# Prasaya/brax

Measured on AMD Instinct MI355X. Metric: env-steps/sec (Ant, 4096 envs/GPU), higher is better.
Workload: dtype f32

## Files before the change

brax_amd/csrc/bx_mix.h:

```cpp
#pragma once
#include <hip/hip_runtime.h>
#include <stdint.h>

namespace bx {

__host__ __device__ __forceinline__ uint64_t mix64(uint64_t seed, uint64_t i) {
  uint64_t z = seed * 0x9E3779B97F4A7C15ull + i + 0x632BE59BD9B4E019ull;
  z = (z ^ (z >> 30)) * 0xBF58476D1CE4E5B9ull;
  z = (z ^ (z >> 27)) * 0x94D049BB133111EBull;
  return z ^ (z >> 31);
}

}
```

brax_amd/csrc/pbd_kernels.hip:

```cpp
#pragma once
#include <hip/hip_runtime.h>
#include <stdint.h>
#include <stdlib.h>
#include <string.h>

#include <type_traits>

#include "bx_mix.h"
#include "pbd_features.h"
#include "pbd_launch.h"
#include "pbd_layout.h"
#include "pbd_math.h"
#include "pbd_stamps.h"

namespace bx {

struct Cst {
  const uint32_t* __restrict__ w;
  __device__ __forceinline__ int i(int off) const { return (int)w[off]; }
  __device__ __forceinline__ float f(int off) const { return __uint_as_float(w[off]); }
  __device__ __forceinline__ v3 f3(int off) const { return mk(f(off), f(off + 1), f(off + 2)); }
};

struct BodyC {
// ... 3399 lines not shown
      for (; i < e && (c.i(H.o_cl + i) >> 24) == g; i++) {
        const float* s = E.cslot + (c.i(H.o_cl + i) & 0xFFFFFF) * SLOT_STRIDE;
        gv = gv + ld3(s);
        ga = ga + ld3(s + 3);
        cnt += s[7];
      }
      float d = 1e-8f + cnt;
      dv = dv + gv / d;
      da = da + ga / d;
    }
    float* acc = E.acc + b * ACC_STRIDE;
    st3(acc + ACC_ICV, dv);
    st3(acc + ACC_ICA, da);
  }
  esync<L>();
}


template <int L>
__device__ void joint_angles(const Cst& c, const BlobHdr& H, const Env& E, int lane,
                             const JointC* hj = nullptr) {
  for (int j = lane; j < H.J; j += L) {
    JointC Jc = hj ? *hj : load_joint(c, H, j);
    QP p = ldqp(E.qp + Jc.bp * QP_STRIDE), q = ldqp(E.qp + Jc.bc * QP_STRIDE);
    v3 axes[3];
    float ang[3];
    axis_angle<F_ALL>(Jc, p, q, axes, ang);
    v3 dv = p.ang - q.ang;
#pragma unroll
    for (int l = 0; l < 3; l++) {
      if (l < Jc.n_angles) {
        E.ang[Jc.angle_off + l] = ang[l];
        E.ang[H.D + Jc.angle_off + l] = dot(dv, axes[l]);
      }
    }
  }
}

__device__ __forceinline__ float clip1(float x) { return clampn(x, -1.f, 1.f); }

__device__ __forceinline__ float euler_z(const float* q) {
  return atan2f(-2.f * q[1] * q[2] + 2.f * q[0] * q[3],
                q[1] * q[1] + q[0] * q[0] - q[3] * q[3] - q[2] * q[2]);
}

__device__ __forceinline__ float euler_y(const float* q) {
  return asinf(clampn(2.f * q[1] * q[3] + 2.f * q[0] * q[2], -1.f, 1.f));
}

__device__ void humanoid_com(const Cst& c, const BlobHdr& H, const float* qp, v3& com, float& msum,
                             bool n16 = false, const float* lmass = nullptr) {
  v3 acc = mk(0.f, 0.f, 0.f);
  float m = 0.f;
  if (n16) {
#pragma unroll
    for (int b = 0; b < 16; b++) {
      const bool in = b < H.N - 1;
      const int bb = in ? b : 0;
      const float w = in ? (lmass ? lmass[bb] : c.f(H.o_body + bb * BODY_STRIDE + BODY_MASS)) : 0.f;
      acc = acc + w * ld3(qp + bb * QP_STRIDE);
      m += w;
    }
    com = acc / m;
    msum = m;
    return;
  }
  for (int b = 0; b < H.N - 1; b++) {
    float mb = c.f(H.o_body + b * BODY_STRIDE + BODY_MASS);
    acc = acc + mb * ld3(qp + b * QP_STRIDE);
    m += mb;
  }
  com = acc / m;
  msum = m;
}

template <int EK>
__device__ __forceinline__ constexpr bool ek_has(int k) {
  return EK == EK_ANY || (EK == EK_ANT && k == BX_ENV_ANT) ||
         (EK == EK_HUM && (k == BX_ENV_HUMANOID || k == BX_ENV_HUMANOID_STANDUP)) ||
         (EK == EK_CHEETAH && k == BX_ENV_HALFCHEETAH) || (EK == EK_PUSHER && k == BX_ENV_PUSHER);
}
#define KIND_IS(k) (ek_has<EK>(k) && kind == (k))

__device__ __forceinline__ float uniform_at(uint64_t seed, uint64_t i, float lo, float hi) {
  const uint64_t z = mix64(seed, i);
  float u = (float)(z >> 40) * (1.0f / 16777216.0f);
  return lo + (hi - lo) * u;
}

__device__ __forceinline__ void arm_tip(const Env& E, const float* coef, v3& tp, v3& tv) {
  const float* a = E.qp + (int)coef[1] * QP_STRIDE;
  v3 off = rotate(mk(.11f, 0.f, 0.f), q4{a[3], a[4], a[5], a[6]});
  tp = ld3(a) + off;
  tv = ld3(a + 7) + cross(ld3(a + 10), off);
}

template <int EK>
__device__ float obs_elem(const Cst& c, const BlobHdr& H, const Env& E, int kind, int flags, int i,
                          const float* act, int aw, bool valid, const float* coef) {
  const int N = H.N, D = H.D;
  const float* q0 = E.qp;
  const bool loco2d = KIND_IS(BX_ENV_HOPPER) || KIND_IS(BX_ENV_WALKER2D);
  if (flags & BX_OBS_XY) {
    if (KIND_IS(BX_ENV_HALFCHEETAH) || loco2d) {
      if (i == 0) return q0[0];
      i -= 1;
    } else {
      if (i < 2) return q0[i];
      i -= 2;
    }
  }
  if (KIND_IS(BX_ENV_ANT)) {
    if (i == 0) return q0[2];
    i -= 1;
    if (i < 4) return q0[3 + i];
    i -= 4;
    if (i < D) return E.ang[i];
    i -= D;
    if (i < 3) return q0[7 + i];
    i -= 3;
    if (i < 3) return q0[10 + i];
    i -= 3;
    if (i < D) return E.ang[D + i];
    i -= D;
    if (i < 3 * N) return clip1(E.acc[(i / 3) * ACC_STRIDE + ACC_ICV + i % 3]);
    i -= 3 * N;
    return clip1(E.acc[(i / 3) * ACC_STRIDE + ACC_ICA + i % 3]);
  }
  if (loco2d) {
    if (i == 0) return q0[2];
    if (i == 1) return euler_y(q0 + 3);
    i -= 2;
    if (i < D) return E.ang[i];
    i -= D;
    if (i == 0) return q0[7];
    if (i == 1) return q0[9];
    if (i == 2) return q0[11];
    i -= 3;
    return E.ang[D + i];
  }
  if (KIND_IS(BX_ENV_INVERTED_PENDULUM)) {
    if (i == 0) return q0[0];
    i -= 1;
    if (i < D) return E.ang[i];
    i -= D;
    if (i == 0) return q0[7];
    return E.ang[D + i - 1];
  }
  if (KIND_IS(BX_ENV_INVERTED_DOUBLE_PENDULUM)) {
    if (i == 0) return q0[0];
    i -= 1;
    if (i < D) return sinf(E.ang[i]);
    i -= D;
    if (i < D) return cosf(E.ang[i]);
    i -= D;
    if (i == 0) return q0[7];
    return E.ang[D + i - 1];
  }
  if (KIND_IS(BX_ENV_ACROBOT)) return E.ang[i];
  if (KIND_IS(BX_ENV_REACHER) || KIND_IS(BX_ENV_REACHERANGLE)) {
    if (i < D) return cosf(E.ang[i]);
    i -= D;
    if (i < D) return sinf(E.ang[i]);
    i -= D;
    const float* tq = E.qp + (int)coef[0] * QP_STRIDE;
    if (i < 2) return tq[i];
    i -= 2;
    v3 tp, tv;
    arm_tip(E, coef, tp, tv);
    if (i < 2) return i == 0 ? tv.x : tv.y;
// ... 201 lines not shown
          o[k] = clip1(a[ACC_ICV + k]);
          o[3 * N + k] = clip1(a[ACC_ICA + k]);
        }
      }
    return;
  }
  if constexpr (EK == EK_HUM && L <= 64) {
    const int N = H.N, D = H.D, M = N - 1;
    const int x = (flags & BX_OBS_XY) ? 2 : 0;
    const float* q0 = E.qp;
    for (int l = lane; l < x + 11; l += L) {
      const int k = l - x;
      float v = l < x ? q0[l] : (k < 5 ? q0[2 + k] : q0[7 + (k - 5)]);
      obs_out[k < 5 ? l : x + 5 + D + (k - 5)] = v;
    }
    for (int j = lane; j < D; j += L) {
      obs_out[x + 5 + j] = E.ang[j];
      obs_out[x + 11 + D + j] = E.ang[D + j];
    }
    const int base = x + 11 + 2 * D;
    const v3 com = ld3(E.red + 32);
    const float msum = E.red[35];
    BX_OST(2);
    for (int b = lane; b < M; b += L) {
      const int ob = H.o_body + b * BODY_STRIDE;
      const float mb = hbody ? hbody->mass : c.f(ob + BODY_MASS);
      const float Ia[3] = {hbody ? hbody->I.x : c.f(ob + BODY_I),
                           hbody ? hbody->I.y : c.f(ob + BODY_I + 1),
                           hbody ? hbody->I.z : c.f(ob + BODY_I + 2)};
      const v3 d = ld3(E.qp + b * QP_STRIDE) - com;
      const v3 vb = ld3(E.qp + b * QP_STRIDE + 7);
      const float nn = norm(d);
      const float dd[3] = {d.x, d.y, d.z};
      float* o = obs_out + base + 9 * b;
#pragma unroll
      for (int r = 0; r < 3; r++)
#pragma unroll
        for (int cc = 0; cc < 3; cc++) {
          float v = mb * (float)(r == cc) * (nn * nn);
          v += (r == cc ? Ia[r] : 0.f) - dd[r] * dd[cc];
          o[3 * r + cc] = v;
        }
      float* ov = obs_out + base + 9 * M + 3 * b;
      ov[0] = mb * vb.x / msum;
      ov[1] = mb * vb.y / msum;
      ov[2] = mb * vb.z / msum;
      const v3 cr = cross(d, vb);
      const float den = 1e-7f + nn * nn;
      float* oa = obs_out + base + 12 * M + 3 * b;
      oa[0] = cr.x / den;
      oa[1] = cr.y / den;
      oa[2] = cr.z / den;
    }
    BX_OST(3);
    const bool ha = lane < H.K;
    ActC A{};
    int dof = 0;
    if (ha && hact && hj) {
      A = *hact;
      dof = hj->dof;
    } else if (ha) {
      A = load_act(c, H, lane);
      dof = c.i(H.o_joint + A.joint * JOINT_STRIDE + J_DOF);
    }
    int off = dof;
    constexpr int W = L < 64 ? L : 64;
#pragma unroll
    for (int sh = 1; sh < W; sh <<= 1) {
      int t = __shfl_up(off, sh, W);
      if ((lane % W) >= sh) off += t;
    }
    off -= dof;
    float* oq = obs_out + base + 15 * M + off;
#pragma unroll
    for (int i = 0; i < 3; i++)
      if (i < dof) oq[i] = (act ? E.arow[take_idx(A.idx[i], aw)] : 0.f) * A.strength;
    BX_OST(4);
    return;
  }
  for (int i = lane; i < obs_size; i += L)
    obs_out[i] = obs_elem<EK>(c, H, E, kind, flags, i, act, aw, act != nullptr, coef);
}




#if defined(BX_WAVES1)
#define BX_STEP_ATTR __attribute__((amdgpu_waves_per_eu(1, 1)))
#else
#define BX_STEP_ATTR
#endif

template <int MODE>
__device__ __forceinline__ float* stage_constants(const uint32_t* blob, const BlobHdr& H,
                                                  float* smem, Cst& c) {
  if constexpr (MODE == MODE_LDS) {
    uint32_t* cl = reinterpret_cast<uint32_t*>(smem);
    for (int i = threadIdx.x; i < H.const_words; i += blockDim.x) cl[i] = blob[i];
    __syncthreads();
    c.w = cl;
    return smem + H.const_words;
  } else {
    c.w = blob;
    return smem;
  }
}

template <int L, int MODE, int F, int M>
__device__ __forceinline__ void system_step_body(const StepArgs& A) {
  extern __shared__ __attribute__((aligned(16))) float smem[];
  BlobHdr H = *reinterpret_cast<const BlobHdr*>(A.blob);
  Cst c{A.blob};
  float* ebase = stage_constants<MODE>(A.blob, H, smem, c);
  constexpr bool S = MODE == MODE_SINGLE;
  constexpr bool MU = MODE == MODE_MULTI;
  const int lane = MU ? (int)threadIdx.x : (int)(threadIdx.x % L);
  const int le = MU ? 0 : (int)(threadIdx.x / L);
  const int64_t e = (int64_t)blockIdx.x * (MU ? 1 : (blockDim.x / L)) + le;
  const bool valid = e < A.n_envs;
  Env E = carve(ebase + le * H.env_words, H, MU);
  zero_slots(E, H, lane);
  Hoist<M, cl_width<F, M>()> X;
  if constexpr (S) {
    load_hoist<M, (F & F_JH) != 0, (F & F_R2) != 0, cl_width<F, M>()>(A.blob + H.o_lane, H, lane, X);
    stage_lim<L, F>(A.blob + H.o_lane, H, E, lane);
  }
  for (int b = lane; b < H.N; b += L) {
    if (valid) {
      load_qp_global(A.qin, e, b, E.qp + b * QP_STRIDE);
    } else {
      float* s = E.qp + b * QP_STRIDE;
      for (int k = 0; k < 13; k++) s[k] = k == 3 ? 1.f : 0.f;
    }
  }
  esync<L>();
  if constexpr (MU) {
    HoistM X;
    load_hoist_multi<L, (F & F_JH) != 0>(c, H, lane, X);
    if (H.o_bimg != 0) {
      const uint32_t* bg = c.w + H.o_bimg;
      for (int k = lane; k < BI_WORDS * H.R; k += L) E.bimg[k] = bg[k];
      const uint4* cg = reinterpret_cast<const uint4*>(c.w + H.o_cen);
      for (int k = lane; k < 2 * H.n_cen + H.n_mat + H.N; k += L) E.cen[k] = cg[k];
    }
    for (int r = lane; r <= H.R; r += L) E.sidx[r] = (uint16_t)0xFFFFu;
    esync<L>();
    const int64_t ro = valid ? e * H.info_rows : 0;
    RowInfoOut io{A.info.contact_pos ? A.info.contact_pos + ro * 3 : nullptr,
                  A.info.contact_normal ? A.info.contact_normal + ro * 3 : nullptr,
                  A.info.contact_penetration ? A.info.contact_penetration + ro : nullptr,
                  A.info.contact_cell ? A.info.contact_cell + ro : nullptr};
    pbd_step_multi<L, F>(c, H, E, lane, valid, valid ? A.act + e * A.act_stride : nullptr,
                         (int)A.act_width, X, io,
                         A.movf ? A.movf + (valid ? e : 0) * (int64_t)(H.R - MCBUF) * MOVF_W : nullptr);
  } else if constexpr (S) {
    v3 icv, ica, iaa;
    pbd_step_single<L, F, M>(c, H, E, lane, valid, valid ? A.act + e * A.act_stride : nullptr,
                             (int)A.act_width, X, icv, ica,
                       iaa);
  } else if (H.spring) {
    spring_step<L, F>(c, H, E, lane, valid, valid ? A.act + e * A.act_stride : nullptr, (int)A.act_width);
  } else {
    pbd_step<L, F>(c, H, E, lane, valid, valid ? A.act + e * A.act_stride : nullptr, (int)A.act_width);
  }
  if (!valid) return;
  for (int b = lane; b < H.N; b += L) {
// ... 58 lines not shown
__device__ __forceinline__ float pol_tanh(float x) { return is_nan(x) ? x : tanhf(x); }
__device__ __forceinline__ float pol_softplus(float x) {
  const float r = fmaxf(x, 0.f) + log1pf(expf(-fabsf(x)));
  return is_nan(x) ? x : r;
}
__device__ __forceinline__ float pol_act(float x, int fn) {
  if (fn == BX_POLICY_RELU) return is_nan(x) ? x : fmaxf(x, 0.f);
  if (fn == BX_POLICY_TANH) return pol_tanh(x);
  const float r = x / (1.f + expf(-x));
  return is_nan(x) ? x : r;
}
template <int L>
__device__ __forceinline__ void pol_layer(const float* W, const float* hin, float* hout, int n_in,
                                          int n_out, int lane, int fn) {
  const float* b = W + n_in * n_out;
  for (int j = lane; j < n_out; j += L) {
    float s0 = b[j], s1 = 0.f, s2 = 0.f, s3 = 0.f;
    const float* w = W + j;
    int i = 0;
#pragma unroll 4
    for (; i + 4 <= n_in; i += 4) {
      const f32x4 h = ld4a(hin + i);
      s0 = fmaf(h.x, w[(i + 0) * n_out], s0);
      s1 = fmaf(h.y, w[(i + 1) * n_out], s1);
      s2 = fmaf(h.z, w[(i + 2) * n_out], s2);
      s3 = fmaf(h.w, w[(i + 3) * n_out], s3);
    }
    for (; i < n_in; i++) s0 = fmaf(hin[i], w[i * n_out], s0);
    const float s = (s0 + s1) + (s2 + s3);
    hout[j] = fn < 0 ? s : pol_act(s, fn);
  }
}
template <int L, bool POP = false>
__device__ __forceinline__ float* policy_eval(const PolArgs& Q, const float* W, const float* pobs,
                                              float* b0, float* b1, int lane, int64_t el, int64_t e,
                                              bool valid, int t, int aw, int64_t n_envs, int head = 0) {
  const float* hin = pobs;
  if (Q.mean) {
    for (int i = lane; i < Q.width[0]; i += L) {
      const float o = pobs[i];
      const float r = (o - Q.mean[i]) / Q.std[i];
      b0[i] = is_nan(o) ? o : r;
    }
    hin = b0;
    esync<L>();
  }
  float* hout = hin == b0 ? b1 : b0;
  for (int l = 0; l < Q.n_layers; l++) {
    const int n_in = Q.width[l], n_out = Q.width[l + 1];
    pol_layer<L>(W, hin, hout, n_in, n_out, lane, l + 1 < Q.n_layers ? Q.act_fn : -1);
    W += (n_in + 1) * n_out;
    esync<L>();
    hin = hout;
    hout = hin == b0 ? b1 : b0;
  }
  if constexpr (POP) {
    if (head == 1) return const_cast<float*>(hin);
  }
  const bool has_scale = Q.width[Q.n_layers] >= 2 * aw;
  for (int a = lane; a < aw; a += L) {
    const float loc = hin[a];
    float scale = 1.f, eps = 0.f;
    if (has_scale) scale = pol_softplus(hin[aw + a]) + Q.min_std;
    if (!Q.det)
      eps = normal_at(Q.seed, Q.offset + (uint64_t)t * Q.step + ((uint64_t)el * (uint64_t)aw + (uint64_t)a) * 2u);
    const float raw = Q.det ? loc : fmaf(scale, eps, loc);
    const float act = pol_tanh(raw);
    const float lp = -0.5f * eps * eps - 0.91893853320467274178f - logf(scale) -
                     2.f * (0.69314718055994530942f - raw - pol_softplus(-2.f * raw));
    hout[a] = act;
    hout[aw + a] = lp;
    if (valid && Q.raw_out) Q.raw_out[((int64_t)t * n_envs + e) * aw + a] = raw;
  }
  esync<L>();
  if (lane == 0 && valid && Q.logp_out) {
    float s = 0.f;
    for (int a = 0; a < aw; a++) s += hout[aw + a];
    Q.logp_out[(int64_t)t * n_envs + e] = s;
  }
  return hout;
}

template <int L, int MODE, int F, int M, int EK = EK_ANY, bool PK = false, bool ONE = false,
          bool POL = false, bool EVL = false, bool POP = false, bool ZH = true>
__device__ __forceinline__ void env_step_body(const EnvArgs& A, const PolArgs& Q = PolArgs{},
                                              const EvalArgs& V = EvalArgs{},
                                              const PopArgs& N = PopArgs{}) {
  static_assert(!EVL || (PK && !ONE), "the evaluation kernels run on the packed K-step layout");
  static_assert(!POP || (POL && EVL), "the population kernels are evaluation kernels with a policy");
  BX_KSTAMP_DECL
  extern __shared__ __attribute__((aligned(16))) float smem[];
  constexpr bool EARLY = PK && ONE && MODE == MODE_SINGLE;
  f32x4 eq0 = {0.f, 0.f, 0.f, 0.f}, eq1 = eq0, eq2 = eq0;
  float eq3 = 0.f;
  if constexpr (EARLY) {
    const int64_t es = A.in.qp.pos.env_stride;
    const int nb = (int)(es >> 4);
    const int ln = (int)(threadIdx.x % L);
    const int64_t ee = (int64_t)blockIdx.x * (blockDim.x / L) + threadIdx.x / L;
    const float* qs = A.in.qp.pos.ptr + (ee < A.n_envs ? ee : 0) * es + (int64_t)(ln < nb ? ln : 0) * 16;
    eq0 = ld4a(qs);
    eq1 = ld4a(qs + 4);
    eq2 = ld4a(qs + 8);
    eq3 = qs[12];
  }
  float ed = 0.f, est = 0.f, ea0 = 0.f, ea1 = 0.f;
  if constexpr (EARLY) {
    const int ln = (int)(threadIdx.x % L);
    const int64_t ee = (int64_t)blockIdx.x * (blockDim.x / L) + threadIdx.x / L;
    const int64_t eel = ee < A.n_envs ? ee : 0;
    ed = A.in.done[eel];
    if (A.in.steps) est = A.in.steps[eel];
    const int aw0 = (int)A.act_width;
    constexpr int C0 = L < 64 ? L : 64;
    if (!A.draw && aw0 > 0 && ln < C0) {
      const float* ar = A.act + eel * A.act_stride;
      ea0 = ar[ln < aw0 ? ln : aw0 - 1];
      if (aw0 > C0) ea1 = ar[C0 + ln < aw0 ? C0 + ln : aw0 - 1];
    }
  }
  BlobHdr H = ONE ? A.hdr : *reinterpret_cast<const BlobHdr*>(A.blob);
  Cst c{A.blob};
  float* ebase = stage_constants<MODE>(A.blob, H, smem, c);
  constexpr bool S = MODE == MODE_SINGLE;
  const int lane = threadIdx.x % L;
  const int le = threadIdx.x / L;
  const int64_t e = (int64_t)blockIdx.x * (blockDim.x / L) + le;
  const bool valid = e < A.n_envs;
  Hoist<M, cl_width<F, M>()> X;
  constexpr bool JBK = S && (F & F_JH) != 0 && EK != EK_ANY && (F & F_C16) == 0;
  if constexpr (S && ONE)
    load_hoist<M, (F & F_JH) != 0, (F & F_R2) != 0, cl_width<F, M>(), JBK, JBK && cb_feat(F)>(
        A.lane_img, H, lane, X);
  Env E = carve(ebase + le * H.env_words, H);
  zero_slots(E, H, lane);
  BX_PSTAMP(5);
  const bx_env_params& P = A.P;
  const int kind = P.kind;
  const int aw = (int)A.act_width;
  const int64_t el = valid ? e : 0;
  if constexpr (S && !ONE)
    load_hoist<M, (F & F_JH) != 0, (F & F_R2) != 0, cl_width<F, M>(), JBK, JBK && cb_feat(F)>(
        A.blob + H.o_lane, H, lane, X);
  if constexpr (S) stage_lim<L, F>(ONE ? A.lane_img : A.blob + H.o_lane, H, E, lane);
  if constexpr (S && L == 16 && !JBK)
    E.red[16 + lane] = X.B.mass;
  BX_PSTAMP(6);
  float done_in = EARLY ? ed : A.in.done[el];
  float steps_in = EARLY ? est : (A.in.steps ? A.in.steps[el] : 0.f);
  if (!valid) done_in = steps_in = 0.f;
  uint32_t rng_c = (A.in.rng && valid) ? A.in.rng[e] : 0u;
  constexpr int C = L < 64 ? L : 64;
  const bool drw = POL || A.draw != 0;
  auto draw_at = [&](int t, int i) {
    return uniform_at(A.draw_seed,
                      A.draw_offset + (uint64_t)t * A.draw_step + (uint64_t)el * (uint64_t)aw + (uint64_t)i,
                      A.draw_lo, A.draw_hi);
  };
  const float* arow_g = drw ? nullptr : A.act + el * A.act_stride;
  float a0 = 0.f;
  const float* pw = nullptr;
  float *pobs = nullptr, *pb0 = nullptr, *pb1 = nullptr, *pact = nullptr;
  if constexpr (POL) {
    float* pa = smem + Q.lds_off;
    pw = Q.params;
    if constexpr (POP) pw += el * N.param_stride;
    if (Q.stage) {
      for (int i = threadIdx.x; i < Q.n_params; i += blockDim.x) pa[i] = Q.params[i];
      pw = pa;
      pa += (Q.n_params + 3) & ~3;
      __syncthreads();
    }
    pobs = pa + le * (Q.obs_words + 2 * Q.buf_words);
    pb0 = pobs + Q.obs_words;
    pb1 = pb0 + Q.buf_words;
    for (int i = lane; i < P.obs_size; i += L) pobs[i] = Q.obs_in[el * P.obs_size + i];
    esync<L>();
  }
  float *ev = nullptr, *em = nullptr;
  if constexpr (EVL) {
    const int nm = P.n_metrics;
    ev = smem + V.lds_off + le * V.words;
    em = ev + nm + 3;
    if (lane == 0)
      for (int k = 0; k < nm + 3; k++)
        ev[k] = (V.in && valid) ? V.in[k * A.n_envs + e] : (k == nm + 1 ? 1.f : 0.f);
  }
  float* mom = nullptr;
  if constexpr (POP) {
    float* pp = smem + N.lds_off + le * N.words;
    const int nw = 2 * P.obs_size + 1;
    if (N.mom_out) {
      mom = pp;
      for (int i = lane; i < nw; i += L) mom[i] = (N.mom_in && valid) ? N.mom_in[e * nw + i] : 0.f;
    }
    if (N.stage) {
      float* row = pp + N.row_off;
      for (int i = lane * 4; i < Q.n_params; i += L * 4) st4a(row + i, ld4a(pw + i));
      pw = row;
    }
    esync<L>();
  }
  if (!POL && aw > 0 && lane < C) a0 = drw ? draw_at(0, lane < aw ? lane : aw - 1) : (EARLY ? ea0 : arow_g[lane < aw ? lane : aw - 1]);
  BX_PSTAMP(7);
  if constexpr (S) {
    float qv[13];
    if constexpr (EARLY) {
#pragma unroll
      for (int k = 0; k < 4; k++) {
        qv[k] = eq0[k];
        qv[4 + k] = eq1[k];
        qv[8 + k] = eq2[k];
      }
      qv[12] = eq3;
    } else {
      load_qp_regs(A.in.qp, el, lane < H.N ? lane : 0, qv);
    }
    if (lane < H.N) {
      float* s = E.qp + lane * QP_STRIDE;
#pragma unroll
      for (int k = 0; k < 13; k++) s[k] = valid ? qv[k] : (k == 3 ? 1.f : 0.f);
    }
  } else {
    for (int b = lane; b < H.N; b += L) {
      if (valid) {
        load_qp_global(A.in.qp, e, b, E.qp + b * QP_STRIDE);
      } else {
        float* s = E.qp + b * QP_STRIDE;
        for (int k = 0; k < 13; k++) s[k] = k == 3 ? 1.f : 0.f;
      }
    }
  }
  BX_PSTAMP(8);
  constexpr bool CBH = ZH && JBK && cbh_feat(F);
  FrozenB Z{};
  auto freeze = [&]() {
    if (X.hasB) {
      Z = load_frozen(E.qp + X.R.b * QP_STRIDE);
      held(Z.b.pos); held(Z.b.rot); held(Z.b.vel); held(Z.b.ang);
      held(Z.n);
    }
  };
  if constexpr (CBH) {
    esync<L>();
    init_frozen_records(H, E, lane);
    freeze();
  }
  const int nst = ONE ? 1 : (A.n_steps > 1 ? A.n_steps : 1);
  for (int t = 0; t < nst; t++) {
  const bool last = !EVL || t == nst - 1;
  const float* act = (valid && !drw) ? A.act + e * A.act_stride + t * A.act_step : nullptr;
  if constexpr (POP) {
    if (mom) {
      const int no = P.obs_size;
      const float w = ev[P.n_metrics + 1];
      for (int i = lane; i < no; i += L) {
        const float o = pobs[i];
        const float d = Q.mean ? o - Q.mean[i] : o;
        float q = d * d;
        asm("" : "+v"(q));
        mom[i] += w * d;
        mom[no + i] += w * q;
      }
      if (lane == 0) mom[2 * no] += w;
    }
  }
  if constexpr (POL) {
    pact = policy_eval<L, POP>(Q, pw, pobs, pb0, pb1, lane, el, e, valid, t, aw, A.n_envs, POP ? N.head : 0);
    esync<L>();
  } else if (t > 0) {
    if (drw) {
      if (aw > 0 && lane < C) a0 = draw_at(t, lane < aw ? lane : aw - 1);
    } else {
      arow_g = A.act + el * A.act_stride + t * A.act_step;
      if (aw > 0 && lane < C) a0 = arow_g[lane < aw ? lane : aw - 1];
    }
  }
  bx_env_state O;
  float* blk = nullptr;
  if constexpr (PK) {
    const int64_t B = A.n_envs;
    blk = EVL ? A.out.qp.pos.ptr : A.out.qp.pos.ptr + t * A.out_step;
    O.obs = blk + B * H.N * 16;
    O.reward = O.obs + B * P.obs_size;
    O.done = O.reward + B;
    O.steps = O.reward + 2 * B;
    O.truncation = O.reward + 3 * B;
    O.metrics = P.n_metrics > 0 ? O.reward + 4 * B : nullptr;
    O.rng = A.out.rng ? A.out.rng + (EVL ? 0 : t * A.rng_step) : nullptr;
  } else {
    O = A.out;
    if (t > 0) {
      const int64_t os = t * A.out_step;
      O.qp.pos.ptr += os; O.qp.rot.ptr += os; O.qp.vel.ptr += os; O.qp.ang.ptr += os;
      O.obs += os; O.reward += os; O.done += os;
      if (O.metrics) O.metrics += os;
      if (O.steps) O.steps += os;
      if (O.truncation) O.truncation += os;
      if (O.rng) O.rng += t * A.rng_step;
    }
  }
  auto store_out_qp = [&](int b, const float* src) {
    if constexpr (PK) {
      float* d = blk + (e * H.N + b) * 16;
      st4a(d, f32x4{src[0], src[1], src[2], src[3]});
      st4a(d + 4, f32x4{src[4], src[5], src[6], src[7]});
      st4a(d + 8, f32x4{src[8], src[9], src[10], src[11]});
      d[12] = src[12];
    } else {
      store_qp_global(O.qp, e, b, src);
    }
  };
  float sq = 0.f;
  for (int i0 = 0; i0 < aw; i0 += C) {
    const int i = i0 + lane;
    float v = a0;
    if constexpr (POL) {
      v = pact[i < aw ? i : aw - 1];
    } else if (i0 > 0 && lane < C)
      v = drw ? draw_at(t, i < aw ? i : aw - 1) : ((EARLY && i0 == C) ? ea1 : arow_g[i < aw ? i : aw - 1]);
    if (i >= aw || !valid) v = 0.f;
    if (drw && A.act_out && valid && lane < C && i < aw) A.act_out[((int64_t)t * A.n_envs + e) * aw + i] = v;
    if constexpr (EK == EK_ANT && L == 16) {
      if (i < H.act_read) E.arow[i] = v;
      sq += row_sum16(v * v);
      continue;
    }
    if (lane < C) {
      E.red[lane] = v;
      if (i < H.act_read) E.arow[i] = v;
    }
    esync<L>();
    if (POL && lane == 0) {
      if (i0 == 0) {
        float r1 = E.red[1] * E.red[1];
        asm("" : "+v"(r1));
        sq = __builtin_fmaf(E.red[0], E.red[0], r1);
#pragma unroll
        for (int k = 2; k < C; k++) sq = __builtin_fmaf(E.red[k], E.red[k], sq);
      } else {
#pragma unroll
        for (int k = 0; k < C; k++) sq = __builtin_fmaf(E.red[k], E.red[k], sq);
      }
    } else if (lane == 0) {
#pragma unroll
      for (int k = 0; k < C; k++) sq += E.red[k] * E.red[k];
    }
    esync<L>();
  }
  esync<L>();
  float steps = 0.f;
  if (valid && (A.in.steps || t > 0)) steps = (P.auto_reset && done_in != 0.f) ? 0.f : steps_in;
  float done = P.auto_reset ? 0.f : done_in;
  float reward_sum = 0.f;
  const int reps = P.episode_length > 0 ? (P.action_repeat > 0 ? P.action_repeat : 1) : 1;
  BX_KSTAMP(10);
  v3 icv = mk(0.f, 0.f, 0.f);
  for (int rep = 0; rep < reps; rep++) {
    v3 pos0 = ld3(E.qp);
    v3 com0 = mk(0.f, 0.f, 0.f);
    float msum = 0.f;
    if (KIND_IS(BX_ENV_HUMANOID) || KIND_IS(BX_ENV_SWIMMER))
      humanoid_com(c, H, E.qp, com0, msum, S && EK == EK_HUM && (F & F_JH) == 0,
                   S && L == 16 && EK == EK_HUM && (F & F_JH) == 0 ? E.red + 16 : nullptr);
    if ((KIND_IS(BX_ENV_UR5E) || KIND_IS(BX_ENV_FETCH)) && lane == 0)
      st3(E.red + 36, ld3(E.qp + (int)P.coef[0] * QP_STRIDE));
    float near0 = 0.f, dist0 = 0.f;
    if (KIND_IS(BX_ENV_PUSHER)) {
      v3 tip = ld3(E.qp + (int)P.coef[0] * QP_STRIDE), obj = ld3(E.qp + (int)P.coef[1] * QP_STRIDE);
      v3 goal = ld3(E.qp + (int)P.coef[2] * QP_STRIDE);
      near0 = -norm(obj - tip);
      dist0 = -norm(obj - goal);
    }
    const float* sact = valid ? E.arow : nullptr;
    int saw = aw;
    float* xact = E.xact;
    if (KIND_IS(BX_ENV_REACHERANGLE)) {
      if (valid && lane < aw) xact[lane] = P.coef[2 + lane] + P.coef[4 + lane] * ((act[lane] + 1.f) / 2.f);
      sact = valid ? xact : nullptr;
    } else if (KIND_IS(BX_ENV_SWIMMER)) {
      const float* q = E.qp + lane * QP_STRIDE;
      q4 rot{0.f, 0.f, 0.f, 0.f};
      v3 vel = mk(0.f, 0.f, 0.f);
      if (lane < 3) {
        rot = q4{q[3], q[4], q[5], q[6]};
        vel = ld3(q + 7);
        v3 lv = rotate(vel, quat_inv(rot));
        float l = lane == 0 ? lv.x : (lane == 1 ? lv.y : lv.z);
        E.red[60 + lane] = P.coef[3 + lane] * fabsf(l) * l;
      }
      esync<L>();
      if (lane < 3 && valid) {
        v3 f = vel * P.coef[2] - mk(E.red[60], E.red[61], E.red[62]);
        f = rotate(f, rot);
        xact[aw + 3 * lane] = clampf(f.x, -5.f, 5.f);
        xact[aw + 3 * lane + 1] = clampf(f.y, -5.f, 5.f);
        xact[aw + 3 * lane + 2] = clampf(f.z, -5.f, 5.f);
      }
      if (valid && lane < aw) xact[lane] = act[lane];
      sact = valid ? xact : nullptr;
      saw = aw + 9;
    } else if (KIND_IS(BX_ENV_GRASP)) {
      for (int i = lane; i < aw; i += L)
        if (valid) xact[i] = P.act_map[i] + P.act_map[aw + i] * ((act[i] + 1.f) / 2.f);
      esync<L>();
      if (lane == 0 && valid) {
        float* pp = E.qp + (int)P.coef[0] * QP_STRIDE;
        v3 palm = ld3(pp);
        v3 d = mk(xact[aw - 3], xact[aw - 2], xact[aw - 1]) - palm;
        float nrm = norm(d);
        float scl = nrm > 2.f ? 2.f / nrm : 1.f;
        st3(pp, palm + scl * d * .15f);
      }
      sact = valid ? xact : nullptr;
    }
    esync<L>();
    if constexpr (S) {
      v3 ica, iaa;
      pbd_step_single<L, F, M, EK != EK_ANY, true, false, CBH>(c, H, E, lane, valid, sact, saw, X, icv,
                                                               ica, iaa, Z);
    } else if (H.spring) {
      spring_step<L, F>(c, H, E, lane, valid, sact, saw);
    } else {
      pbd_step<L, F>(c, H, E, lane, valid, sact, saw);
    }
    BX_KSTAMP(11);
    env_observe<L, EK>(c, H, E, lane, kind, P.obs_flags, P.obs_size, act, aw,
                   (valid && (POL || last)) ? (POL ? pobs : O.obs + e * P.obs_size) : nullptr, P.coef, S ? &X.J : nullptr,
                   (S && !JBK) ? &X.B : nullptr, (S && EK == EK_HUM) ? &X.A : nullptr);
    BX_KSTAMP(12);
    float ccs = 0.f;
    if constexpr (S && EK == EK_ANT && L == 16) {
      const v3 cv = mk(clip1(icv.x), clip1(icv.y), clip1(icv.z));
      ccs = row_sum16(X.own ? cv.x * cv.x + cv.y * cv.y + cv.z * cv.z : 0.f);
    }
    if (lane == 0 && valid) {
      const float dt = H.dt;
      float* m = EVL ? (P.n_metrics > 0 ? em : nullptr) : (O.metrics ? O.metrics + e * P.n_metrics : nullptr);
      v3 p1 = ld3(E.qp);
      float reward = 0.f;
      if (KIND_IS(BX_ENV_ANT)) {
        v3 vel = (p1 - pos0) / dt;
        float fwd = vel.x;
        float z = p1.z;
        float healthy = in_range_or_nan(z, P.coef[4], P.coef[5]) ? 1.f : 0.f;
        bool term = P.coef[6] != 0.f;
        float hr = term ? P.coef[3] : P.coef[3] * healthy;
        float ctrl = P.coef[1] * sq;
        float cs = ccs;
        if constexpr (!(S && EK == EK_ANT && L == 16))
          for (int b = 0; b < H.N; b++)
            for (int k = 0; k < 3; k++) {
              float cv = clip1(E.acc[b * ACC_STRIDE + ACC_ICV + k]);
              cs += cv * cv;
            }
        float ccost = P.coef[2] * cs;
        reward = fwd + hr - ctrl - ccost;
        done = term ? 1.f - healthy : 0.f;
        if (m) {
          m[0] = norm(p1); m[1] = fwd; m[2] = -ccost; m[3] = -ctrl; m[4] = fwd;
          m[5] = hr; m[6] = p1.x; m[7] = vel.x; m[8] = p1.y; m[9] = vel.y;
        }
      } else if (KIND_IS(BX_ENV_HALFCHEETAH)) {
        float v0 = (p1.x - pos0.x) / dt;
        float fwd = P.coef[0] * v0;
        float ctrl = P.coef[1] * sq;
        reward = fwd - ctrl;
        if (m) { m[0] = -ctrl; m[1] = fwd; m[2] = p1.x; m[3] = v0; }
      } else if (KIND_IS(BX_ENV_HUMANOID)) {
        v3 com1 = ld3(E.red + 32);
        v3 v = (com1 - com0) / dt;
        float fwd = P.coef[0] * v.x;
        float z = p1.z;
        float healthy = in_range_or_nan(z, P.coef[4], P.coef[5]) ? 1.f : 0.f;
        bool term = P.coef[6] != 0.f;
        float hr = term ? P.coef[3] : P.coef[3] * healthy;
        float ctrl = P.coef[1] * sq;
        reward = fwd + hr - ctrl;
        done = term ? 1.f - healthy : 0.f;
        if (m) {
          m[0] = norm(com1); m[1] = fwd; m[2] = hr; m[3] = fwd; m[4] = -ctrl;
          m[5] = com1.x; m[6] = v.x; m[7] = com1.y; m[8] = v.y;
        }
      } else if (KIND_IS(BX_ENV_HOPPER) || KIND_IS(BX_ENV_WALKER2D)) {
        float xv = (p1.x - pos0.x) / dt;
        float fwd = P.coef[0] * xv;
        float ay = euler_y(E.qp + 3);
        float z = p1.z;
        float healthy = in_range_or_nan(z, P.coef[3], P.coef[4]) &&
                        in_range_or_nan(ay, P.coef[5], P.coef[6]) ? 1.f : 0.f;
        bool term = P.coef[7] != 0.f;
        float hr = term ? P.coef[2] : P.coef[2] * healthy;
        float ctrl = P.coef[1] * sq;
        reward = fwd + hr - ctrl;
        done = term ? 1.f - healthy : 0.f;
        if (m) { m[0] = -ctrl; m[1] = fwd; m[2] = hr; m[3] = p1.x; m[4] = xv; }
      } else if (KIND_IS(BX_ENV_INVERTED_PENDULUM)) {
        reward = 1.f;
        done = fabsf(E.ang[0]) > .2f && !is_nan(E.ang[0]) ? 1.f : 0.f;
      } else if (KIND_IS(BX_ENV_INVERTED_DOUBLE_PENDULUM)) {
        const float* q2 = E.qp + 2 * QP_STRIDE;
        v3 tip = ld3(q2) + rotate(mk(0.f, 0.f, .3f), q4{q2[3], q2[4], q2[5], q2[6]});
        float x = tip.x, y = tip.z;
        float dist = 0.01f * (x * x) + (y - 2.f) * (y - 2.f);
        float v1 = E.ang[H.D], v2 = E.ang[H.D + 1];
        float velp = 1e-3f * (v1 * v1) + 5e-3f * (v2 * v2);
        reward = 10.f - dist - velp;
        done = y <= 1.f && !is_nan(y) ? 1.f : 0.f;
      } else if (KIND_IS(BX_ENV_ACROBOT)) {
        float a0 = E.ang[0], a1 = E.ang[1], w0 = E.ang[H.D], w1 = E.ang[H.D + 1];
        float dist = a0 * a0 + a1 * a1;
        float velp = 1e-3f * (w0 * w0 + w1 * w1);
        reward = 10.f - dist - velp;
        done = 0.f;
        if (m) { m[0] = 0.f; m[1] = dist; m[2] = reward; m[3] = velp; }
      } else if (KIND_IS(BX_ENV_REACHER) || KIND_IS(BX_ENV_REACHERANGLE)) {
        v3 tp, tv;
        arm_tip(E, P.coef, tp, tv);
        float rd = -norm(tp - ld3(E.qp + (int)P.coef[0] * QP_STRIDE));
        if (KIND_IS(BX_ENV_REACHER)) {
          float rc = -sq;
// ... 32 lines not shown
          v3 up = rotate(mk(0.f, 0.f, 1.f), tr);
          float is_up = .1f * dt * dot(up, mk(0.f, 0.f, 1.f));
          float height = .1f * dt * E.qp[2];
          float facing = dot(dir, rotate(mk(1.f, 0.f, 0.f), tr));
          float whit = hit * facing;
          reward = height + moving + is_up + whit;
          if (m) { m[0] = hit; m[1] = moving; m[2] = height; m[3] = is_up; m[4] = whit; }
        }
        const uint32_t key = rng_c + (uint32_t)rep;
        if (rep == reps - 1 && last) O.rng[e] = key + 1u;
        if (hit != 0.f) {
          float u0 = uniform_at(key, 0, 0.f, 1.f), u1 = uniform_at(key, 1, 0.f, 1.f);
          float rr = P.coef[2] + P.coef[3] * u0;
          float an = 3.14159265358979323846f * 2.f * u1;
          float* g = E.qp + gi * QP_STRIDE;
          g[0] = rr * cosf(an);
          g[1] = rr * sinf(an);
          g[2] = P.coef[4];
        }
      } else if (KIND_IS(BX_ENV_GRASP)) {
        const int oi = (int)P.coef[1], gi = (int)P.coef[2], hi = (int)P.coef[3];
        v3 op = ld3(E.qp + oi * QP_STRIDE), hp = ld3(E.qp + (int)P.coef[0] * QP_STRIDE);
        v3 hv = ld3(E.qp + hi * QP_STRIDE + 7);
        v3 rel = op - hp;
        float od = norm(rel);
        float planar = norm(mul(rel, mk(1.f, 1.f, 0.f)));
        v3 odir = rel / (1e-6f + od);
        float mto = .1f * dt * dot(hv, odir);
        float close = .1f * dt * 1.f / (1.f + planar);
        v3 trel = ld3(E.qp + gi * QP_STRIDE) - op;
        float td = norm(trel);
        v3 tdir = trel / (1e-6f + td);
        float mtt = 1.5f * dt * dot(ld3(E.qp + oi * QP_STRIDE + 7), tdir);
        float touch = 0.f;
        const int tb[4] = {3, 9, 12, 15};
        for (int k = 0; k < 4; k++) {
          const float* cv = E.acc + tb[k] * ACC_STRIDE + ACC_ICV;
          touch += cv[0] * cv[0] + cv[1] * cv[1] + cv[2] * cv[2] > 0.00001f ? 1.f : 0.f;
        }
        touch = 0.2f * dt * touch;
        float hit = td < P.coef[4] ? 1.f : 0.f;
        reward = mto + close + touch + 5.f * hit + mtt;
        if (m) { m[0] = close; m[1] = hit; m[2] = mtt; m[3] = mto; m[4] = touch; }
        const uint32_t key = rng_c + (uint32_t)rep;
        if (rep == reps - 1 && last) O.rng[e] = key + 1u;
        if (hit != 0.f) {
          float u0 = uniform_at(key, 0, 0.f, 1.f), u1 = uniform_at(key, 1, 0.f, 1.f);
          float u2 = uniform_at(key, 2, 0.f, 1.f);
          float rr = P.coef[4] + P.coef[5] * u0;
          float an = 3.14159265358979323846f * 2.f * u1;
          float* g = E.qp + gi * QP_STRIDE;
          g[0] = rr * cosf(an);
          g[1] = rr * sinf(an);
          g[2] = P.coef[6] * u2;
        }
      } else if (KIND_IS(BX_ENV_PUSHER)) {
        float rc = -sq;
        reward = dist0 + 0.1f * rc + 0.5f * near0;
        if (m) { m[0] = rc; m[1] = dist0; m[2] = near0; }
      } else if (KIND_IS(BX_ENV_HUMANOID_STANDUP)) {
        float uph = (p1.z - 0.f) / dt;
        float ctrl = P.coef[1] * sq;
        reward = uph + 1.f - ctrl;
        if (m) { m[0] = uph; m[1] = -ctrl; }
      }
      reward_sum = rep == 0 ? reward : reward_sum + reward;
      E.red[0] = done;
    }
    esync<L>();
  }
  BX_KSTAMP(13);
  done = E.red[0];
  float trunc = 0.f;
  bool reset_now = false;
  if (P.episode_length > 0) {
    steps = steps + (float)reps;
    float ep = (float)P.episode_length;
    float d_inner = done;
    done = steps >= ep ? 1.f : d_inner;
    trunc = steps >= ep ? 1.f - d_inner : 0.f;
  }
  if (P.auto_reset) reset_now = done != 0.f;
  if (valid) {
    if (lane == 0 && last) {
      O.reward[e] = reward_sum;
      O.done[e] = done;
      if (O.steps) O.steps[e] = steps;
      if (O.truncation) O.truncation[e] = trunc;
    }
    if constexpr (EVL) {
      if (lane == 0) {
        const int nm = P.n_metrics;
        const float active = ev[nm + 1];
        if (active != 0.f) ev[nm + 2] = steps;
        for (int k = 0; k < nm; k++) ev[k] += em[k] * active;
        if constexpr (POP) ev[nm] += (reward_sum - N.reward_shift) * active;
        else ev[nm] += reward_sum * active;
        ev[nm + 1] = active * (1.f - done);
        if (last) {
          for (int k = 0; k < nm; k++) O.metrics[e * nm + k] = em[k];
          for (int k = 0; k < nm + 3; k++) V.out[k * A.n_envs + e] = ev[k];
        }
      }
    }
    if constexpr (POP) {
      if (last && mom) {
        const int nw = 2 * P.obs_size + 1;
        for (int i = lane; i < nw; i += L) N.mom_out[e * nw + i] = mom[i];
      }
    }
    if (reset_now) {
      for (int b = lane; b < H.N; b += L) {
        float tmp[13];
        load_qp_global(P.first_qp, e, b, tmp);
        if (last) store_out_qp(b, tmp);
        if (t + 1 < nst) {
          float* s = E.qp + b * QP_STRIDE;
#pragma unroll
          for (int k = 0; k < 13; k++) s[k] = tmp[k];
        }
      }
      for (int i = lane; i < P.obs_size; i += L) {
        const float fo = P.first_obs[e * P.obs_size + i];
        if (last) O.obs[e * P.obs_size + i] = fo;
        if constexpr (POL) pobs[i] = fo;
      }
    } else if (last) {
      for (int b = lane; b < H.N; b += L) store_out_qp(b, E.qp + b * QP_STRIDE);
      if constexpr (POL)
        for (int i = lane; i < P.obs_size; i += L) O.obs[e * P.obs_size + i] = pobs[i];
    }
  }
  done_in = done;
  steps_in = steps;
  rng_c += (uint32_t)reps;
  esync<L>();
  if constexpr (CBH) {
    if (valid && reset_now && t + 1 < nst) freeze();
  }
  }
  BX_KSTAMP(14);
}



template <int L, int MODE, int F, int M, int EK = EK_ANY>
__global__ void __launch_bounds__(L > 64 ? L : 64) BX_STEP_ATTR env_step_kernel(EnvArgs A) {
  env_step_body<L, MODE, F, M, EK>(A);
}

}
```

brax_amd/csrc/pbd_single.hip:

```cpp
#define BX_TU_FAST
#include <hip/hip_runtime.h>
#include <stdint.h>

#include "pbd_dispatch.h"
#include "pbd_kernels.hip"
#include "pbd_launch.h"
#include "pbd_stamps.h"

namespace bx {

template <int L, int MODE, int F, int M, int EK = EK_ANY>
__global__ void __launch_bounds__(L > 64 ? L : 64) BX_STEP_ATTR env_step_packed_kernel(EnvArgs A) {
  env_step_body<L, MODE, F, M, EK, true, true>(A);
}
template <int L, int MODE, int F, int M, int EK = EK_ANY>
__global__ void __launch_bounds__(L > 64 ? L : 64) __attribute__((amdgpu_waves_per_eu(2)))
env_step_wide_kernel(EnvArgs A) {
  env_step_body<L, MODE, F, M, EK>(A);
}
template <int L, int MODE, int F, int M, int EK = EK_ANY>
__global__ void __launch_bounds__(L > 64 ? L : 64) __attribute__((amdgpu_waves_per_eu(2)))
env_rollout_wide_kernel(EnvArgs A) {
  env_step_body<L, MODE, F, M, EK, true>(A);
}
template <int L, int MODE, int F, int M, int EK = EK_ANY>
__global__ void __launch_bounds__(L > 64 ? L : 64) BX_STEP_ATTR env_rollout_kernel(EnvArgs A) {
  env_step_body<L, MODE, F, M, EK, true>(A);
}

#define BX_SYSTEM_STEP_CASE(VL, VF, VM, UNUSED) \
  case single_key(VL, VF, VM): launch_one(system_step_kernel<VL, 1, VF, VM>, grid, tpb, lds, s, a); break;
hipError_t launch_system_step_single(int L, int feat, int gw, int tpb, int64_t n_envs, size_t lds,
                                     hipStream_t s, const StepArgs& a) {
  const dim3 grid = single_grid(L, tpb, n_envs);
  const SingleVariant v = single_variant(L, feat, gw);
  switch (single_key(v.L, v.F, v.M)) {
    BX_SINGLE_VARIANTS(BX_SYSTEM_STEP_CASE, 0)
    default: return hipErrorInvalidValue;
  }
  return hipGetLastError();
}

struct StepFamily {
  static constexpr EnvFamily id = FAM_STEP;
  template <int L, int F, int M, int EK>
  static auto kernel(const EnvArgs& a, bool wide) -> void (*)(EnvArgs) {
    const StepKernel k = step_kernel(KindVariant{F, M, EK}, wide, a.n_steps, a.packed != 0);
    if constexpr (EK == EK_ANT) {
      if (k == K_ROLLOUT_WIDE) return env_rollout_wide_kernel<L, 1, F, M, EK>;
      if (k == K_STEP_WIDE) return env_step_wide_kernel<L, 1, F, M, EK>;
    }
    if constexpr (has_rollout_kernel(F, EK))
      if (k == K_ROLLOUT) return env_rollout_kernel<L, 1, F, M, EK>;
    if (k == K_STEP_PACKED) return env_step_packed_kernel<L, 1, F, M, EK>;
    return env_step_kernel<L, 1, F, M, EK>;
  }
};
hipError_t launch_env_step_single(int L, int feat, int gw, int tpb, int64_t n_envs, size_t lds,
                                  hipStream_t s, const EnvArgs& a, int fold) {
  return launch_env_family<StepFamily>(L, feat, gw, tpb, n_envs, lds, s, fold, a);
}
__global__ void __launch_bounds__(64) partner_kernel(float* out, int lanes) {
  const float v = (float)threadIdx.x;
  out[threadIdx.x] = lanes == 16 ? xh(v) : v;
}
hipError_t debug_partner(float* out64, int lanes, hipStream_t s) {
  hipLaunchKernelGGL(partner_kernel, dim3(1), dim3(64), 0, s, out64, lanes);
  return hipGetLastError();
}
hipError_t debug_stamps(unsigned long long* out, int reset) {
#ifdef BX_STAMPS
  return stamps_readback(HIP_SYMBOL(bx_stamp_wave), out, reset, (reset & 4) != 0);
#else
  (void)out;
  (void)reset;
  return hipErrorNotSupported;
#endif
}

}
```

Before: 200.3 million.

## Strength-reduce Ant rollout output addressing and RNG with running per-step offsets

Adds a running-tail mode to the open-loop Ant rollout kernel. Per-lane output offsets (qp, obs, scalars, metrics, action record) are computed once as 32-bit byte offsets and advanced each step instead of being recomputed with 64-bit multiplies. The splitmix RNG start state is also carried and bumped by draw_step, so only the finish mix runs per step. Ant observations are stored directly via a specialized store routine. This cuts per-step integer and address arithmetic and register pressure, but it relies on 32-bit offsets not overflowing and on obs layout assumptions specific to Ant.

```diff
diff --git a/brax_amd/csrc/bx_mix.h b/brax_amd/csrc/bx_mix.h
--- a/brax_amd/csrc/bx_mix.h
+++ b/brax_amd/csrc/bx_mix.h
@@ -4,11 +4,16 @@
 
 namespace bx {
 
-__host__ __device__ __forceinline__ uint64_t mix64(uint64_t seed, uint64_t i) {
-  uint64_t z = seed * 0x9E3779B97F4A7C15ull + i + 0x632BE59BD9B4E019ull;
+__host__ __device__ __forceinline__ uint64_t mix64_start(uint64_t seed, uint64_t i) {
+  return seed * 0x9E3779B97F4A7C15ull + i + 0x632BE59BD9B4E019ull;
+}
+__host__ __device__ __forceinline__ uint64_t mix64_finish(uint64_t z) {
   z = (z ^ (z >> 30)) * 0xBF58476D1CE4E5B9ull;
   z = (z ^ (z >> 27)) * 0x94D049BB133111EBull;
   return z ^ (z >> 31);
 }
+__host__ __device__ __forceinline__ uint64_t mix64(uint64_t seed, uint64_t i) {
+  return mix64_finish(mix64_start(seed, i));
+}
 
 }
diff --git a/brax_amd/csrc/pbd_kernels.hip b/brax_amd/csrc/pbd_kernels.hip
--- a/brax_amd/csrc/pbd_kernels.hip
+++ b/brax_amd/csrc/pbd_kernels.hip
@@ -3505,10 +3505,12 @@
 }
 #define KIND_IS(k) (ek_has<EK>(k) && kind == (k))
 
-__device__ __forceinline__ float uniform_at(uint64_t seed, uint64_t i, float lo, float hi) {
-  const uint64_t z = mix64(seed, i);
+__device__ __forceinline__ float uniform_of(uint64_t z, float lo, float hi) {
   float u = (float)(z >> 40) * (1.0f / 16777216.0f);
   return lo + (hi - lo) * u;
+}
+__device__ __forceinline__ float uniform_at(uint64_t seed, uint64_t i, float lo, float hi) {
+  return uniform_of(mix64(seed, i), lo, hi);
 }
 
 __device__ __forceinline__ void arm_tip(const Env& E, const float* coef, v3& tp, v3& tv) {
@@ -3876,6 +3878,42 @@
     obs_out[i] = obs_elem<EK>(c, H, E, kind, flags, i, act, aw, act != nullptr, coef);
 }
 
+struct RollTail {
+  char* blk;
+  char* arec;
+  uint32_t q;
+  uint32_t row;
+  uint32_t ot, oj, ov, oc, oa;
+  uint32_t sc, met, act;
+  const float* tsrc;
+  bool ton;
+};
+__device__ __forceinline__ float* tail_at(char* base, uint32_t off) {
+  asm volatile("" : "+v"(off));
+  return reinterpret_cast<float*>(base + off);
+}
+template <int L>
+__device__ __forceinline__ void ant_observe_store(const BlobHdr& H, const Env& E, int lane,
+                                                  const RollTail& T, bool forces) {
+  const int N = H.N, D = H.D;
+  if (T.ton) *tail_at(T.blk, T.ot) = *T.tsrc;
+  for (int j = lane, o = 0; j < D; j += L, o += 4 * L) {
+    *tail_at(T.blk, T.oj + o) = E.ang[j];
+    *tail_at(T.blk, T.ov + o) = E.ang[D + j];
+  }
+  if (forces)
+    for (int b = lane, o = 0; b < N; b += L, o += 12 * L) {
+      const float* a = E.acc + b * ACC_STRIDE;
+      float* ov = tail_at(T.blk, T.oc + o);
+      float* oa = tail_at(T.blk, T.oa + o);
+#pragma unroll
+      for (int k = 0; k < 3; k++) {
+        ov[k] = clip1(a[ACC_ICV + k]);
+        oa[k] = clip1(a[ACC_ICA + k]);
+      }
+    }
+}
+
 
 
 
@@ -4100,12 +4138,14 @@
 }
 
 template <int L, int MODE, int F, int M, int EK = EK_ANY, bool PK = false, bool ONE = false,
-          bool POL = false, bool EVL = false, bool POP = false, bool ZH = true>
+          bool POL = false, bool EVL = false, bool POP = false, bool ZH = true, bool RT = false>
 __device__ __forceinline__ void env_step_body(const EnvArgs& A, const PolArgs& Q = PolArgs{},
                                               const EvalArgs& V = EvalArgs{},
                                               const PopArgs& N = PopArgs{}) {
   static_assert(!EVL || (PK && !ONE), "the evaluation kernels run on the packed K-step layout");
   static_assert(!POP || (POL && EVL), "the population kernels are evaluation kernels with a policy");
+  static_assert(!RT || (PK && !ONE && !POL && !EVL && MODE == MODE_SINGLE && EK == EK_ANT && L == 16),
+                "the running tail is the open-loop Ant rollout kernel's");
   BX_KSTAMP_DECL
   extern __shared__ __attribute__((aligned(16))) float smem[];
   constexpr bool EARLY = PK && ONE && MODE == MODE_SINGLE;
@@ -4177,6 +4217,32 @@
   };
   const float* arow_g = drw ? nullptr : A.act + el * A.act_stride;
   float a0 = 0.f;
+  uint64_t dz = 0;
+  RollTail T{};
+  if constexpr (RT) {
+    const int lc = lane < aw ? lane : aw - 1;
+    dz = mix64_start(A.draw_seed, A.draw_offset + (uint64_t)el * (uint64_t)aw + (uint64_t)lc);
+    const int N = H.N, D = H.D, O = P.obs_size;
+    const int x = (P.obs_flags & BX_OBS_XY) ? 2 : 0;
+    const uint32_t Bn = (uint32_t)A.n_envs, en = (uint32_t)el;
+    T.blk = reinterpret_cast<char*>(A.out.qp.pos.ptr);
+    T.arec = reinterpret_cast<char*>(A.act_out);
+    T.q = 4u * ((en * N + (lane < N ? lane : 0)) * 16);
+    const uint32_t orow = Bn * N * 16 + en * O;
+    T.row = 4u * (orow + lane);
+    const int k = lane - x;
+    T.ton = lane < x + 11;
+    T.tsrc = E.qp + (lane < x ? lane : (k < 5 ? 2 + k : 7 + (k - 5)));
+    T.ot = 4u * (orow + (k < 5 ? lane : x + 5 + D + (k - 5)));
+    T.oj = 4u * (orow + x + 5 + lane);
+    T.ov = 4u * (orow + x + 11 + D + lane);
+    T.oc = 4u * (orow + x + 11 + 2 * D + 3 * lane);
+    T.oa = T.oc + 4u * (3 * N);
+    const uint32_t osc = Bn * (N * 16 + O);
+    T.sc = 4u * (osc + en);
+    T.met = 4u * (osc + 4 * Bn + en * P.n_metrics);
+    T.act = 4u * (en * aw + lane);
+  }
   const float* pw = nullptr;
   float *pobs = nullptr, *pb0 = nullptr, *pb1 = nullptr, *pact = nullptr;
   if constexpr (POL) {
@@ -4286,6 +4352,14 @@
   if constexpr (POL) {
     pact = policy_eval<L, POP>(Q, pw, pobs, pb0, pb1, lane, el, e, valid, t, aw, A.n_envs, POP ? N.head : 0);
     esync<L>();
+  } else if (RT && t > 0) {
+    if (drw) {
+      dz += A.draw_step;
+      if (aw > 0 && lane < C) a0 = uniform_of(mix64_finish(dz), A.draw_lo, A.draw_hi);
+    } else {
+      arow_g += A.act_step;
+      if (aw > 0 && lane < C) a0 = arow_g[lane < aw ? lane : aw - 1];
+    }
   } else if (t > 0) {
     if (drw) {
       if (aw > 0 && lane < C) a0 = draw_at(t, lane < aw ? lane : aw - 1);
@@ -4296,7 +4370,9 @@
   }
   bx_env_state O;
   float* blk = nullptr;
-  if constexpr (PK) {
+  if constexpr (RT) {
+    O = bx_env_state{};
+  } else if constexpr (PK) {
     const int64_t B = A.n_envs;
     blk = EVL ? A.out.qp.pos.ptr : A.out.qp.pos.ptr + t * A.out_step;
     O.obs = blk + B * H.N * 16;
@@ -4320,7 +4396,7 @@
   }
   auto store_out_qp = [&](int b, const float* src) {
     if constexpr (PK) {
-      float* d = blk + (e * H.N + b) * 16;
+      float* d = RT ? tail_at(T.blk, T.q) : blk + (e * H.N + b) * 16;
       st4a(d, f32x4{src[0], src[1], src[2], src[3]});
       st4a(d + 4, f32x4{src[4], src[5], src[6], src[7]});
       st4a(d + 8, f32x4{src[8], src[9], src[10], src[11]});
@@ -4338,7 +4414,9 @@
     } else if (i0 > 0 && lane < C)
       v = drw ? draw_at(t, i < aw ? i : aw - 1) : ((EARLY && i0 == C) ? ea1 : arow_g[i < aw ? i : aw - 1]);
     if (i >= aw || !valid) v = 0.f;
-    if (drw && A.act_out && valid && lane < C && i < aw) A.act_out[((int64_t)t * A.n_envs + e) * aw + i] = v;
+    if constexpr (RT) {
+      if (drw && A.act_out && valid && lane < C && i < aw) *tail_at(T.arec, T.act + 4 * i0) = v;
+    } else if (drw && A.act_out && valid && lane < C && i < aw) A.act_out[((int64_t)t * A.n_envs + e) * aw + i] = v;
     if constexpr (EK == EK_ANT && L == 16) {
       if (i < H.act_read) E.arow[i] = v;
       sq += row_sum16(v * v);
@@ -4444,8 +4522,10 @@
     }
     BX_KSTAMP(11);
     env_observe<L, EK>(c, H, E, lane, kind, P.obs_flags, P.obs_size, act, aw,
-                   (valid && (POL || last)) ? (POL ? pobs : O.obs + e * P.obs_size) : nullptr, P.coef, S ? &X.J : nullptr,
+                   (!RT && valid && (POL || last)) ? (POL ? pobs : O.obs + e * P.obs_size) : nullptr, P.coef, S ? &X.J : nullptr,
                    (S && !JBK) ? &X.B : nullptr, (S && EK == EK_HUM) ? &X.A : nullptr);
+    if constexpr (RT)
+      if (valid) ant_observe_store<L>(H, E, lane, T, P.coef[7] != 0.f);
     BX_KSTAMP(12);
     float ccs = 0.f;
     if constexpr (S && EK == EK_ANT && L == 16) {
@@ -4454,7 +4534,9 @@
     }
     if (lane == 0 && valid) {
       const float dt = H.dt;
-      float* m = EVL ? (P.n_metrics > 0 ? em : nullptr) : (O.metrics ? O.metrics + e * P.n_metrics : nullptr);
+      float* m = EVL ? (P.n_metrics > 0 ? em : nullptr)
+                 : RT ? (P.n_metrics > 0 ? tail_at(T.blk, T.met) : nullptr)
+                      : (O.metrics ? O.metrics + e * P.n_metrics : nullptr);
       v3 p1 = ld3(E.qp);
       float reward = 0.f;
       if (KIND_IS(BX_ENV_ANT)) {
@@ -4653,7 +4735,15 @@
   }
   if (P.auto_reset) reset_now = done != 0.f;
   if (valid) {
-    if (lane == 0 && last) {
+    if constexpr (RT) {
+      if (lane == 0) {
+        const uint32_t B4 = 4u * (uint32_t)A.n_envs;
+        *tail_at(T.blk, T.sc) = reward_sum;
+        *tail_at(T.blk, T.sc + B4) = done;
+        *tail_at(T.blk, T.sc + 2 * B4) = steps;
+        *tail_at(T.blk, T.sc + 3 * B4) = trunc;
+      }
+    } else if (lane == 0 && last) {
       O.reward[e] = reward_sum;
       O.done[e] = done;
       if (O.steps) O.steps[e] = steps;
@@ -4693,6 +4783,10 @@
       }
       for (int i = lane; i < P.obs_size; i += L) {
         const float fo = P.first_obs[e * P.obs_size + i];
+        if constexpr (RT) {
+          *tail_at(T.blk, T.row + 4 * (i - lane)) = fo;
+          continue;
+        }
         if (last) O.obs[e * P.obs_size + i] = fo;
         if constexpr (POL) pobs[i] = fo;
       }
@@ -4705,6 +4799,10 @@
   done_in = done;
   steps_in = steps;
   rng_c += (uint32_t)reps;
+  if constexpr (RT) {
+    T.blk += 4 * A.out_step;
+    T.arec += 4 * A.n_envs * aw;
+  }
   esync<L>();
   if constexpr (CBH) {
     if (valid && reset_now && t + 1 < nst) freeze();
diff --git a/brax_amd/csrc/pbd_single.hip b/brax_amd/csrc/pbd_single.hip
--- a/brax_amd/csrc/pbd_single.hip
+++ b/brax_amd/csrc/pbd_single.hip
@@ -25,7 +25,8 @@
 }
 template <int L, int MODE, int F, int M, int EK = EK_ANY>
 __global__ void __launch_bounds__(L > 64 ? L : 64) BX_STEP_ATTR env_rollout_kernel(EnvArgs A) {
-  env_step_body<L, MODE, F, M, EK, true>(A);
+  constexpr bool RT = EK == EK_ANT && L == 16 && MODE == MODE_SINGLE;
+  env_step_body<L, MODE, F, M, EK, true, false, false, false, false, true, RT>(A);
 }
 
 #define BX_SYSTEM_STEP_CASE(VL, VF, VM, UNUSED) \
```

New measurement: 204.2 million (median of 6 runs). +1.9%, better.
